# Huvinesh-Rajendran-12/keras-geometric

Hardware: AMD Instinct MI355X
Metric: aggregated edges/sec + achieved HBM GB/s, GCNConv fwd, 1/2/4/8 MI355X (higher is better)
Workload: dtype fp32; 1 GPU; GCNConv fwd, R-MAT 10000000 nodes / 100000000 edges (+self loops), normalized, bias, F 128->128; nodes=10000000, edges=100000000, nodes_per_gpu=10000000, e_agg_per_gpu=110000000, max_in_degree=138539, mode=split-hub, fused aggregate->transform (W on bf16x3-split MFMA, f32-accurate), parallelism=single

## Files before the change

### include/kgx.h

```cpp
#ifndef KGX_H_
#define KGX_H_

#include <stddef.h>
#include <stdint.h>

#ifdef __cplusplus
extern "C" {
#endif

typedef void* kgx_stream_t;

enum kgx_status {
  KGX_OK = 0,
  KGX_ERR_ARG = 1,
  KGX_ERR_HIP = 2,
  KGX_ERR_INDEX = 3,
  KGX_ERR_UNSUPPORTED = 4
};

enum kgx_reduce { KGX_SUM = 0, KGX_MEAN = 1, KGX_MAX = 2, KGX_MIN = 3, KGX_STD = 4 };

enum kgx_epilogue { KGX_EPI_NONE = 0, KGX_EPI_BIAS = 1, KGX_EPI_GIN = 2, KGX_EPI_RAW = 3, KGX_EPI_ACCUM = 4 };

enum kgx_csr_flags {
// ... 92 lines not shown
int kgx_spmm_gemm_ex(int reduce, const int32_t* rowptr, const int32_t* rows, int64_t n_rows,
                     const int32_t* items, int64_t n_items, int64_t n_long_items, const int32_t* split,
                     int64_t n_split, const int32_t* idx, const float* w, const float* x, int64_t ld_x,
                     int64_t F_in, const float* W, int64_t F_out, const float* bias, int flags,
                     float gin_scale, float* out, int64_t ld_out, float* partials, float* agg_out,
                     int64_t ld_agg, kgx_stream_t stream);

int kgx_spmm_gemm_ex2(int reduce, const int32_t* rowptr, const int32_t* rows, int64_t n_rows,
                      const int32_t* items, int64_t n_items, int64_t n_long_items, int64_t n_short_end,
                      const int32_t* tiny_pack, const float* tiny_w, int64_t n_tiny_deg2,
                      const int32_t* split, int64_t n_split,
                      const int32_t* idx, const float* w, const float* x, int64_t ld_x, int64_t F_in,
                      const float* W, int64_t F_out, const float* bias, int flags, float gin_scale, float* out,
                      int64_t ld_out, float* partials, float* agg_out, int64_t ld_agg, kgx_stream_t stream);

int kgx_spmm_gemm_ex3(int reduce, const int32_t* rowptr, const int32_t* rows, int64_t n_rows,
                      const int32_t* items, int64_t n_items, int64_t n_long_items, int64_t n_short_end,
                      const int32_t* tiny_pack, const float* tiny_w, int64_t n_tiny_deg2,
                      const int32_t* split, int64_t n_split, const int32_t* idx, const float* w,
                      const float* x, int64_t ld_x, const float* x2, int64_t n_x1, int64_t F_in,
                      const float* W, int64_t F_out, const float* bias, int flags, float gin_scale, float* out,
                      int64_t ld_out, float* partials, float* agg_out, int64_t ld_agg, kgx_stream_t stream);

int kgx_spmm_gemm_f256(int reduce, const int32_t* rowptr, const int32_t* rows, int64_t n_rows,
                       const int32_t* items, int64_t n_items, int64_t n_long_items, int64_t n_short_end,
                       const int32_t* tiny_pack, const float* tiny_w, const int32_t* split, int64_t n_split,
                       const int32_t* idx, const float* w, const float* x, int64_t ld_x, int64_t F_in,
                       const float* W, int64_t F_out, const float* bias, int flags, float gin_scale,
                       float* out, int64_t ld_out, float* partials, float* agg_out, int64_t ld_agg,
                       kgx_stream_t stream);

int kgx_spmm_gemm_f256_ex(int reduce, const int32_t* rowptr, const int32_t* rows, int64_t n_rows,
                          const int32_t* items, int64_t n_items, int64_t n_long_items, int64_t n_short_end,
                          const int32_t* tiny_pack, const float* tiny_w, const int32_t* split, int64_t n_split,
                          const int32_t* idx, const float* w, const float* x, int64_t ld_x, const float* x2,
                          int64_t n_x1, int64_t F_in, const float* W, int64_t F_out, const float* bias, int flags,
                          float gin_scale, float* out, int64_t ld_out, float* partials, float* agg_out,
                          int64_t ld_agg, kgx_stream_t stream);

int kgx_gemm_tn_workspace_bytes(int64_t N, int64_t K, int64_t M, size_t* bytes);
int kgx_gemm_tn(int64_t N, const float* P, int64_t ldp, int64_t K, const float* D, int64_t ldd, int64_t M,
                float* dW, int64_t ld_dw, float* db, void* workspace, size_t workspace_bytes,
                kgx_stream_t stream);

int kgx_spmm_max_backward(int reduce, int raw, const int32_t* rowptr, int64_t n_rows, const int32_t* idx,
                          const float* table, int64_t ld_table, int64_t F,
// ... 94 lines not shown
```

### keras-geometric_amd/csrc/kgx_internal.h

```cpp
#pragma once

#include <hip/hip_runtime.h>

#include <cstdarg>
#include <cstdint>
#include <cstdio>

#include <cstdlib>
#include <cstring>
#include <mutex>
#include <vector>

#include "kgx.h"

namespace kgx {

void set_error(const char* fmt, ...);

inline hipStream_t as_stream(kgx_stream_t s) { return reinterpret_cast<hipStream_t>(s); }

inline int ceil_log2_u64(uint64_t v) {
  int b = 0;
  while ((uint64_t(1) << b) < v) ++b;
  return b;
// ... 198 lines not shown
  hipStream_t s = nullptr;
  hipError_t fork(CuSplit* c, hipStream_t caller) {
    hipError_t e = hipEventRecord(c->fork, caller);
    if (e == hipSuccess) e = hipStreamWaitEvent(c->head, c->fork, 0);
    if (e == hipSuccess) e = hipStreamWaitEvent(c->tail, c->fork, 0);
    if (e != hipSuccess) return e;
    cs = c;
    s = caller;
    return hipSuccess;
  }
  hipError_t join() {
    if (!cs) return hipSuccess;
    CuSplit* c = cs;
    cs = nullptr;
    const hipError_t e[4] = {hipEventRecord(c->jh, c->head), hipEventRecord(c->jt, c->tail),
                             hipStreamWaitEvent(s, c->jh, 0), hipStreamWaitEvent(s, c->jt, 0)};
    for (hipError_t v : e)
      if (v != hipSuccess) return v;
    return hipSuccess;
  }
  ~SplitJoin() { (void)join(); }
};


inline int next_pow2(int v) {
  int p = 1;
  while (p < v) p <<= 1;
  return p;
}
inline int log2i(int v) {
  int l = 0;
  while ((1 << l) < v) ++l;
  return l;
}

}

#define KGX_CHECK_HIP(expr)                                                      \
  do {                                                                           \
    hipError_t kgx_e_ = (expr);                                                  \
    if (kgx_e_ != hipSuccess) {                                                  \
      kgx::set_error("%s:%d: %s failed: %s", __FILE__, __LINE__, #expr,          \
                     hipGetErrorString(kgx_e_));                                 \
      return KGX_ERR_HIP;                                                        \
    }                                                                            \
  } while (0)
// ... 11 lines not shown
```

### keras-geometric_amd/csrc/spmm_gemm.hip

```cpp
#include <cstdlib>
#include <type_traits>

#include "kgx_bf16x3.h"
#include "kgx_internal.h"
#include "kgx_mfma.h"
#include "kgx_red.h"
#include "kgx_vec.h"

namespace kgx {
namespace {

constexpr int kFin = 128;
constexpr int kGroups = 16;
constexpr int kThreads = kGroups * 32;
constexpr int kTileLd = kFin + 4;

constexpr int kFPlanes = 3;

struct FusedArgs {
  const int32_t* rowptr;
  const int32_t* rows;
  int64_t n_rows;
  const int4* items;
  int64_t n_items;
// ... 6 lines not shown
  int64_t ld_x;
  const float* W;
  int F_in;
  int F_out;
  const float* bias;
  float* out;
  int64_t ld_o;
  float* partials;
  float* agg_out;
  int64_t ld_agg;
  int pre_gin;
  int accumulate;
  int share_gpu;
  int relu;
  float gin_scale;
  int64_t n_short_end;
  const int4* tpack;
  const float2* tw;
  int64_t n_tiny;
  int64_t n_tiny2;
  const float* x2b;
  int32_t n_x1;
  bool cu_split;
};


template <bool NARROW, typename Args>
__device__ __forceinline__ void load_w128(const Args& a, bool w_ok, int n_col, int q, bf16x8_t (&wfh)[4],
                                          bf16x8_t (&wfm)[4], bf16x8_t (&wfl)[4]) {
  auto wv = [&](int k) { return w_ok && (!NARROW || k < a.F_in) ? a.W[int64_t(k) * a.F_out + n_col] : 0.0f; };
#pragma unroll
  for (int s = 0; s < 4; ++s) {
    u32x4_t ph, pm, pl;
#pragma unroll
    for (int j = 0; j < 8; j += 2) {
      const float v0 = wv(32 * q + 8 * s + j), v1 = wv(32 * q + 8 * s + j + 1);
      uint32_t h, m_, l;
      split3_pair(v0, v1, h, m_, l);
      ph[j / 2] = h;
      pm[j / 2] = m_;
      pl[j / 2] = l;
    }
    wfh[s] = __builtin_bit_cast(bf16x8_t, ph);
    wfm[s] = __builtin_bit_cast(bf16x8_t, pm);
    wfl[s] = __builtin_bit_cast(bf16x8_t, pl);
  }
// ... 558 lines not shown
        vload<4>(xv, a.x + int64_t(row) * a.ld_x + (!NARROW || lane * 4 < a.F_in ? lane * 4 : 0));
#pragma unroll
        for (int k = 0; k < 4; ++k) acc[k] = __fadd_rn(__fmul_rn(a.gin_scale, xv[k]), acc[k]);
      }
#pragma unroll
      for (int k = 0; k < 4; ++k) vrow[g][lane * 4 + k] = acc[k];
      if (a.agg_out && (!NARROW || lane * 4 < a.F_in)) vstore<4>(a.agg_out + int64_t(row) * a.ld_agg + lane * 4, acc);
    }
    __syncthreads();
    if (row >= 0) {
      for (int c = lane; c < a.F_out; c += 32) {
        float s = 0.0f;
        for (int k = 0; k < (NARROW ? a.F_in : kFin); ++k) s = fmaf(vrow[g][k], a.W[int64_t(k) * a.F_out + c], s);
        float v = s + (a.bias ? a.bias[c] : 0.0f);
        if (a.accumulate) v = __fadd_rn(a.out[int64_t(row) * a.ld_o + c], v);
        if (a.relu) v = fmaxf(v, 0.0f);
        a.out[int64_t(row) * a.ld_o + c] = v;
      }
    }
    __syncthreads();
  }
}

inline int fused_fork_mode() {
  const char* h = getenv("KGX_FUSED_FORK");
  return h ? atoi(h) : 0;
}

inline unsigned fused_grid(const FusedArgs& a, int64_t need, int64_t full) {
  const int64_t cap = a.share_gpu ? shared_cap(full) : full;
  return unsigned(need < cap ? need : cap);
}

template <int RED, bool W, bool TWO, bool NARROW>
int launch_short(const FusedArgs& a, hipStream_t s, int cus) {
  auto k = spmm_gemm_short_kernel<RED, W, TWO, NARROW>;
  const int64_t need = (a.n_short_end - a.n_long + kShortRows - 1) / kShortRows;
  hipLaunchKernelGGL(k, dim3(fused_grid(a, need, occupancy_blocks(k, kThreads, 2, cus))), dim3(kThreads), 0, s, a);
  KGX_CHECK_LAUNCH();
  return KGX_OK;
}

template <int RED, bool W, bool TWO, bool NARROW>
int launch_tiny(const FusedArgs& a, hipStream_t s, int cus) {
  const bool extra = a.pre_gin || a.agg_out;
  for (int part = 0; part < 2; ++part) {
// ... 1 lines not shown
    b.tpack = a.tpack + (part ? a.n_tiny2 : 0);
    b.tw = a.tw ? a.tw + (part ? a.n_tiny2 : 0) : nullptr;
    b.n_tiny = part ? a.n_tiny - a.n_tiny2 : a.n_tiny2;
    if (b.n_tiny <= 0) continue;
    auto k = part ? (extra ? spmm_gemm_tiny_kernel<RED, W, true, 1, TWO, NARROW>
                           : spmm_gemm_tiny_kernel<RED, W, false, 1, TWO, NARROW>)
                  : (extra ? spmm_gemm_tiny_kernel<RED, W, true, 2, TWO, NARROW>
                           : spmm_gemm_tiny_kernel<RED, W, false, 2, TWO, NARROW>);
    const int rows = part ? tiny_rows<1>() : tiny_rows<2>();
    const int64_t need = (b.n_tiny + rows - 1) / rows;
    hipLaunchKernelGGL(k, dim3(fused_grid(a, need, cus > 0 ? cus : cu_count())), dim3(kTinyThreads), 0, s, b);
    KGX_CHECK_LAUNCH();
  }
  return KGX_OK;
}

template <int RED, bool W, bool TWO = false, bool NARROW = false>
int launch(const FusedArgs& a, hipStream_t s) {
  const int64_t work = a.items ? a.n_long : a.n_rows;
  const bool has_short = a.items && a.n_long < a.n_short_end;
  const bool has_tiny = a.tpack && a.n_tiny > 0;
  hipStream_t sh = s, st = s;
  int cus_h = 0, cus_t = 0;
  SplitJoin join;
  if ((a.cu_split || fused_fork_mode() == 3) && work > 0 && (has_tiny || has_short)) {
    const char* e = getenv("KGX_FUSED_CU_SPLIT");
    if (CuSplit* cs = cu_split(e ? atoi(e) : 8, s)) {
      KGX_CHECK_HIP(join.fork(cs, s));
      sh = cs->head;
      st = cs->tail;
      cus_h = cs->n_head;
      cus_t = cs->n_tail;
    }
  }
  auto k = spmm_gemm_kernel<RED, W, TWO, NARROW>;
  auto fk = spmm_gemm_fixup_kernel<RED, NARROW>;
  if (work > 0) {
    const int64_t need = (work + kGroups - 1) / kGroups;
    hipLaunchKernelGGL(k, dim3(fused_grid(a, need, occupancy_blocks(k, kThreads, 2, cus_h))), dim3(kThreads), 0, sh, a);
    KGX_CHECK_LAUNCH();
  }
  if (has_short && launch_short<RED, W, TWO, NARROW>(a, st, cus_t) != KGX_OK) return KGX_ERR_HIP;
  if (has_tiny && launch_tiny<RED, W, TWO, NARROW>(a, st, cus_t) != KGX_OK) return KGX_ERR_HIP;
  if (a.items && a.n_split > 0) {
    const int64_t blocks = (a.n_split + 7) / 8;
    hipLaunchKernelGGL(fk, dim3(unsigned(blocks < 4096 ? blocks : 4096)), dim3(256), 0, sh, a);
    KGX_CHECK_LAUNCH();
  }
  KGX_CHECK_HIP(join.join());
  return KGX_OK;
}

}
}

using namespace kgx;

extern "C" int kgx_spmm_gemm(int reduce, const int32_t* rowptr, const int32_t* rows, int64_t n_rows,
                             const int32_t* items, int64_t n_items, const int32_t* split, int64_t n_split,
                             const int32_t* idx, const float* w, const float* x, int64_t ld_x, int64_t F_in,
                             const float* W, int64_t F_out, const float* bias, int flags, float gin_scale,
                             float* out, int64_t ld_out, float* partials, float* agg_out, int64_t ld_agg,
                             kgx_stream_t stream_) {
  return kgx_spmm_gemm_ex(reduce, rowptr, rows, n_rows, items, n_items, n_items, split, n_split, idx, w, x, ld_x,
                          F_in, W, F_out, bias, flags, gin_scale, out, ld_out, partials, agg_out, ld_agg, stream_);
}
// ... 10 lines not shown
}

extern "C" int kgx_spmm_gemm_ex2(int reduce, const int32_t* rowptr, const int32_t* rows, int64_t n_rows,
                                 const int32_t* items, int64_t n_items, int64_t n_long_items, int64_t n_short_end,
                                 const int32_t* tiny_pack, const float* tiny_w, int64_t n_tiny_deg2,
                                 const int32_t* split,
                                 int64_t n_split, const int32_t* idx, const float* w, const float* x, int64_t ld_x,
                                 int64_t F_in, const float* W, int64_t F_out, const float* bias, int flags,
                                 float gin_scale, float* out, int64_t ld_out, float* partials, float* agg_out,
                                 int64_t ld_agg, kgx_stream_t stream_) {
  return kgx_spmm_gemm_ex3(reduce, rowptr, rows, n_rows, items, n_items, n_long_items, n_short_end, tiny_pack, tiny_w,
                           n_tiny_deg2, split, n_split, idx, w, x, ld_x, nullptr, 0, F_in, W, F_out, bias, flags,
                           gin_scale, out, ld_out, partials, agg_out, ld_agg, stream_);
}

extern "C" int kgx_spmm_gemm_ex3(int reduce, const int32_t* rowptr, const int32_t* rows, int64_t n_rows,
                                 const int32_t* items, int64_t n_items, int64_t n_long_items, int64_t n_short_end,
                                 const int32_t* tiny_pack, const float* tiny_w, int64_t n_tiny_deg2,
                                 const int32_t* split, int64_t n_split, const int32_t* idx, const float* w,
                                 const float* x, int64_t ld_x, const float* x2, int64_t n_x1, int64_t F_in,
                                 const float* W, int64_t F_out, const float* bias, int flags, float gin_scale,
                                 float* out, int64_t ld_out, float* partials, float* agg_out, int64_t ld_agg,
                                 kgx_stream_t stream_) {
  hipStream_t stream = as_stream(stream_);
  KGX_REQUIRE(!x2 || (n_x1 >= 0 && n_x1 < (int64_t(1) << 31) && reinterpret_cast<uintptr_t>(x2) % 16 == 0),
              KGX_ERR_ARG, "kgx_spmm_gemm: x2 must be 16-byte aligned and 0 <= n_x1 < 2^31");
  KGX_REQUIRE(!x2 || (reduce == KGX_SUM && F_in == kFin && F_out % 16 == 0), KGX_ERR_UNSUPPORTED,
              "kgx_spmm_gemm: two-table gathers are implemented for sums at F_in 128, F_out %% 16 == 0 "
              "(the sharded GCN / GIN passes)");
  KGX_REQUIRE(!items || tiny_pack || n_short_end == n_items, KGX_ERR_ARG,
              "kgx_spmm_gemm: without tiny_pack, n_short_end must equal n_items");
  KGX_REQUIRE(!items || (n_long_items >= 0 && n_long_items <= n_short_end && n_short_end <= n_items), KGX_ERR_ARG,
              "kgx_spmm_gemm: need 0 <= n_long_items <= n_short_end <= n_items");
  KGX_REQUIRE(!tiny_pack || (items && (w == nullptr || tiny_w)), KGX_ERR_ARG,
              "kgx_spmm_gemm: the tiny-row records need the schedule (and weights when weighted)");
  KGX_REQUIRE(!tiny_pack || (n_tiny_deg2 >= 0 && n_tiny_deg2 <= n_items - n_short_end), KGX_ERR_ARG,
              "kgx_spmm_gemm: n_tiny_deg2 must lie in [0, n_items - n_short_end]");
  KGX_REQUIRE(reduce >= KGX_SUM && reduce <= KGX_MIN, KGX_ERR_ARG, "kgx_spmm_gemm: reduce %d unsupported", reduce);
  KGX_REQUIRE(F_in > 0 && F_in <= kFin && F_in % 4 == 0, KGX_ERR_UNSUPPORTED,
              "kgx_spmm_gemm: F_in must be a multiple of 4 <= %d (got %lld)", kFin, (long long)F_in);
  KGX_REQUIRE(F_out > 0 && F_out <= 128 && F_out % 4 == 0, KGX_ERR_UNSUPPORTED,
              "kgx_spmm_gemm: F_out must be a multiple of 4 <= 128 (got %lld)", (long long)F_out);
  KGX_REQUIRE(n_rows >= 0 && n_items >= 0 && n_split >= 0, KGX_ERR_ARG, "kgx_spmm_gemm: negative size");
  KGX_REQUIRE((flags & ~(KGX_FUSED_PRE_GIN | KGX_FUSED_ACCUMULATE | KGX_FUSED_SHARE_GPU | KGX_FUSED_RELU |
                         KGX_FUSED_CU_SPLIT)) == 0,
              KGX_ERR_ARG, "kgx_spmm_gemm: unknown flags 0x%x", flags);
// ... 25 lines not shown
  a.n_split = items ? n_split : 0;
  a.idx = idx;
  a.w = w;
  a.x = x;
  a.ld_x = ld_x;
  a.n_x1 = x2 ? int32_t(n_x1) : INT32_MAX;
  a.x2b = x2 ? reinterpret_cast<const float*>(reinterpret_cast<uintptr_t>(x2) -
                                               uintptr_t(n_x1) * uintptr_t(ld_x) * sizeof(float))
             : x;
  a.W = W;
  a.F_in = int(F_in);
  a.F_out = int(F_out);
  a.bias = bias;
  a.out = out;
  a.ld_o = ld_out;
  a.partials = partials;
  a.agg_out = agg_out;
  a.ld_agg = ld_agg;
  a.pre_gin = (flags & KGX_FUSED_PRE_GIN) != 0;
  a.accumulate = (flags & KGX_FUSED_ACCUMULATE) != 0;
  a.share_gpu = (flags & KGX_FUSED_SHARE_GPU) != 0;
  a.relu = (flags & KGX_FUSED_RELU) != 0;
  a.cu_split = (flags & KGX_FUSED_CU_SPLIT) != 0;
  a.gin_scale = gin_scale;
  const bool wt = w != nullptr;
  if (x2) return wt ? launch<KGX_SUM, true, true>(a, stream) : launch<KGX_SUM, false, true>(a, stream);
  if (F_in < kFin || F_out % 16 != 0) {
    switch (reduce) {
      case KGX_SUM: return wt ? launch<KGX_SUM, true, false, true>(a, stream) : launch<KGX_SUM, false, false, true>(a, stream);
      case KGX_MEAN: return wt ? launch<KGX_MEAN, true, false, true>(a, stream) : launch<KGX_MEAN, false, false, true>(a, stream);
      case KGX_MAX: return wt ? launch<KGX_MAX, true, false, true>(a, stream) : launch<KGX_MAX, false, false, true>(a, stream);
      default: return wt ? launch<KGX_MIN, true, false, true>(a, stream) : launch<KGX_MIN, false, false, true>(a, stream);
    }
  }
  switch (reduce) {
    case KGX_SUM: return wt ? launch<KGX_SUM, true>(a, stream) : launch<KGX_SUM, false>(a, stream);
    case KGX_MEAN: return wt ? launch<KGX_MEAN, true>(a, stream) : launch<KGX_MEAN, false>(a, stream);
    case KGX_MAX: return wt ? launch<KGX_MAX, true>(a, stream) : launch<KGX_MAX, false>(a, stream);
    default: return wt ? launch<KGX_MIN, true>(a, stream) : launch<KGX_MIN, false>(a, stream);
  }
}
```

### keras-geometric_amd/keras_geometric_amd/_native.py

```python

from __future__ import annotations

import ctypes
import os
from pathlib import Path

import torch

_PKG_ROOT = Path(__file__).resolve().parent.parent
LIB_PATH = Path(os.environ.get("KGX_LIB", _PKG_ROOT / "lib" / "libkgx.so"))

KGX_OK, KGX_ERR_ARG, KGX_ERR_HIP, KGX_ERR_INDEX, KGX_ERR_UNSUPPORTED = range(5)
SUM, MEAN, MAX, MIN, STD = range(5)
EPI_NONE, EPI_BIAS, EPI_GIN, EPI_RAW, EPI_ACCUM = range(5)
FUSED_PRE_GIN, FUSED_ACCUMULATE, FUSED_SHARE_GPU, FUSED_RELU, FUSED_CU_SPLIT = 1, 2, 4, 8, 16
CSR_SELF_LOOPS, CSR_SEGMENT_ONLY, CSR_GCN_NORM = 1, 2, 4
DENSE_RELU, DENSE_ACCUMULATE = 1, 2
DENSE_MAX_K, DENSE_MAX_N = 256, 256
POOL_SCORE_TANH = 1
POOL_MAX_F = 256
NEG_NO_SELF, NEG_REJECT_EDGES = 1, 2
EDGE_DOT_U = 8

REDUCE_IDS = {"sum": SUM, "mean": MEAN, "max": MAX, "min": MIN, "std": STD}
# ... 67 lines not shown
        _i32p, _f32p, _f32p, _i64, _i64, _f32p, _i64, _f32p, _int, ctypes.c_float,
        _f32p, _i64, _f32p, _f32p, _i64, ctypes.c_void_p,
    ],
    "kgx_spmm_gemm_ex2": [
        _int, _i32p, _i32p, _i64, _i32p, _i64, _i64, _i64, _i32p, _f32p, _i64, _i32p, _i64,
        _i32p, _f32p, _f32p, _i64, _i64, _f32p, _i64, _f32p, _int, ctypes.c_float,
        _f32p, _i64, _f32p, _f32p, _i64, ctypes.c_void_p,
    ],
    "kgx_spmm_gemm_f256": [
        _int, _i32p, _i32p, _i64, _i32p, _i64, _i64, _i64, _i32p, _f32p, _i32p, _i64,
        _i32p, _f32p, _f32p, _i64, _i64, _f32p, _i64, _f32p, _int, ctypes.c_float,
        _f32p, _i64, _f32p, _f32p, _i64, ctypes.c_void_p,
    ],
    "kgx_spmm_gemm_f256_ex": [
        _int, _i32p, _i32p, _i64, _i32p, _i64, _i64, _i64, _i32p, _f32p, _i32p, _i64,
        _i32p, _f32p, _f32p, _i64, _f32p, _i64, _i64, _f32p, _i64, _f32p, _int, ctypes.c_float,
        _f32p, _i64, _f32p, _f32p, _i64, ctypes.c_void_p,
    ],
    "kgx_spmm_gemm_ex3": [
        _int, _i32p, _i32p, _i64, _i32p, _i64, _i64, _i64, _i32p, _f32p, _i64, _i32p, _i64,
        _i32p, _f32p, _f32p, _i64, _f32p, _i64, _i64, _f32p, _i64, _f32p, _int, ctypes.c_float,
        _f32p, _i64, _f32p, _f32p, _i64, ctypes.c_void_p,
    ],
    "kgx_spmm_max_backward": [
        _int, _int, _i32p, _i64, _i32p, _f32p, _i64, _i64, _f32p, _i64, _f32p, _i64, ctypes.c_void_p,
    ],
    "kgx_gatv2_backward": [
        _i32p, _i32p, _i64, _i32p, _i64, _i32p, _i64, _i32p, _f32p, _f32p, _i64, _f32p, _int, _int,
        ctypes.c_float, _f32p, _i64, _f32p, _f32p, _f32p, _i64,
        _i32p, _i32p, _i64, _i32p, _i64, _i32p, _i64, _i32p, _i32p,
        _f32p, _f32p, _i64, _f32p, _f32p, _f32p, _f32p, _i32p, ctypes.c_float, ctypes.c_uint64, ctypes.c_void_p,
    ],
    "kgx_gatv2": [
        _i32p, _i32p, _i64, _i32p, _i64, _i32p, _i64,
        _i32p, _f32p, _f32p, _i64, _f32p, _int, _int, ctypes.c_float,
        _f32p, _i64, _f32p, _f32p, _f32p, _i32p, ctypes.c_float, ctypes.c_uint64, ctypes.c_void_p,
    ],
    "kgx_softmax_pool": [
        _i32p, _i32p, _i64, _i32p, _i64, _i32p, _i64, _i32p, _f32p, _i64, _i64,
        _f32p, _f32p, _f32p, _int, _f32p, _f32p, _i64, _f32p, _f32p, ctypes.c_void_p,
    ],
    "kgx_softmax_pool_backward": [
        _i64, _i64, _i32p, _f32p, _i64, _i64, _f32p, _f32p, _f32p, _i64, _f32p, _i64, _f32p, _i64, _f32p,
        ctypes.c_void_p,
    ],
    "kgx_dense": [
# ... 103 lines not shown
```

### keras-geometric_amd/keras_geometric_amd/ops.py

```python

from __future__ import annotations

import ctypes
import os
import threading
from typing import List, Optional

import torch

from . import _native as nat
from .graph import CSRGraph


def _f32c(t: Optional[torch.Tensor]) -> Optional[torch.Tensor]:
    if t is None:
        return None
    if t.dtype != torch.float32:
        raise TypeError(f"kgx kernels compute in fp32; got {t.dtype}")
    return t.contiguous()


_EXACT_DYN = __import__("os").environ.get("KGX_EXACT_DYN", "1") != "0"


# ... 229 lines not shown
        return True
    idx = dev.index if dev.index is not None else torch.cuda.current_device()
    ok = _DEVICE_SPLIT_OK.get(idx)
    if ok is None:
        ok = _DEVICE_SPLIT_OK[idx] = nat.lib().kgx_cu_split_supported(int(idx)) == 1
    return ok


def _split_allowed(dev: torch.device | None = None) -> bool:
    if _share_gpu() and os.environ.get("KGX_CU_SPLIT_SHARED") != "1":
        return False
    if getattr(_NOSPLIT, "on", False):
        return False
    if dev is not None and dev.type == "cuda" and dev.index is not None and dev.index != torch.cuda.current_device():
        return False
    return _device_split_ok(dev)


def _count_cu_split() -> None:
    global CU_SPLIT_LAUNCHES
    CU_SPLIT_LAUNCHES += 1


def _fused_cu_split(n_edges: int, n_tail_rows: int) -> bool:
    per32 = _per32_override("KGX_FUSED_CU_SPLIT")
    if per32 is not None:
        return n_tail_rows > 0 and per32 > 0
    return n_edges >= 50_000_000 and n_tail_rows >= 2_000_000


def _partial_width(x: torch.Tensor) -> int:
    return F256 if x.shape[1] == F256 else 128


def _fused_launch(out, agg, x, x2, rowptr, rows, items, split, idx, w, n_slots, reduce, W, bias, flags, gin_scale,
                  allow_split, n_long, tpack, tw, n_short_end, n_tiny2, dev):
    n_dst = rowptr.numel() - 1
    n_items = 0 if items is None else items.shape[0]
    n_split = 0 if split is None else split.shape[0]
    partials = None
    if items is not None and n_split > 0:
        partials = torch.empty((n_slots, _partial_width(x)), dtype=torch.float32, device=dev)
    allow_split = allow_split and items is not None
    if x.shape[1] == F256:
        if tpack is not None and allow_split and _split_allowed(dev) and \
                _f256_cu_split(idx.numel(), n_items - (n_short_end if n_short_end >= 0 else n_items)):
            flags |= nat.FUSED_CU_SPLIT
            _count_cu_split()
        _f256_call(reduce, rowptr, rows, n_dst, items, n_items, split, n_split, idx, w, x, x2, W, bias, flags,
                   gin_scale, out, partials, agg, dev, tpack, tw, n_short_end, n_long)
        return
    n_long = n_items if n_long < 0 or n_long > n_items else n_long
    n_se, tpack, tw, n_tiny2 = _tiny_abi(items, n_items, n_long, tpack, tw if w is not None else None, n_short_end,
                                         n_tiny2)
    if allow_split and _split_allowed(dev) and _fused_cu_split(idx.numel(), n_items - n_long):
        flags |= nat.FUSED_CU_SPLIT
        _count_cu_split()
    x2p, n_x1 = _x2_args(x, x2)
    nat.check(
        nat.lib().kgx_spmm_gemm_ex3(
            reduce, nat.ptr(rowptr), nat.ptr(rows), n_dst, nat.ptr(items), n_items, n_long, n_se, nat.ptr(tpack),
            nat.ptr(tw), n_tiny2, nat.ptr(split), n_split,
            nat.ptr(idx), nat.ptr(w), nat.ptr(x), x.stride(0), x2p, n_x1, x.shape[1], nat.ptr(W), W.shape[1],
            nat.ptr(bias), flags, float(gin_scale), nat.ptr(out), out.stride(0), nat.ptr(partials),
            nat.ptr(agg), agg.stride(0) if agg is not None else 0, nat.stream(dev),
        ),
        "kgx_spmm_gemm",
    )


def _spmm_gemm_impl(x, rowptr, rows, items, split, idx, w, n_slots, reduce, W, bias, pre_gin, gin_scale, save_agg,
                    relu=False, n_long=-1, tpack=None, tw=None, n_short_end=-1, n_tiny2=0, x2=None):
    x, w, W, bias, x2 = _f32c(x), _f32c(w), _f32c(W), _f32c(bias), _f32c(x2)
    dev = nat.require_device(x, rowptr, rows, idx, w, W, bias, items, split, x2)
    n_dst = rowptr.numel() - 1
    out = torch.empty((n_dst, W.shape[1]), dtype=torch.float32, device=dev)
    agg = torch.empty((n_dst if save_agg else 0, x.shape[1]), dtype=torch.float32, device=dev)
    if n_dst == 0:
        return out, agg
    flags = int(pre_gin) | (nat.FUSED_SHARE_GPU if _share_gpu() else 0) | (nat.FUSED_RELU if relu else 0)
    _fused_launch(out, agg if save_agg else None, x, x2, rowptr, rows, items, split, idx, w, n_slots, reduce, W, bias,
                  flags, gin_scale, not save_agg, n_long, tpack, tw, n_short_end, n_tiny2, dev)
    return out, agg


@torch.library.custom_op("kgx::spmm_gemm", mutates_args=())
def spmm_gemm(
    x: torch.Tensor,
    rowptr: torch.Tensor,
    rows: torch.Tensor,
    items: Optional[torch.Tensor],
    split: Optional[torch.Tensor],
    idx: torch.Tensor,
    w: Optional[torch.Tensor],
    n_slots: int,
    reduce: int,
    W: torch.Tensor,
    bias: Optional[torch.Tensor],
    pre_gin: bool,
    gin_scale: float,
    relu: bool = False,
    n_long: int = -1,
    tpack: Optional[torch.Tensor] = None,
    tw: Optional[torch.Tensor] = None,
    n_short_end: int = -1,
# ... 545 lines not shown


def multi_aggregate(g: CSRGraph, table: torch.Tensor, reduces, *, by_edge: bool = False,
                    exact: bool = False) -> torch.Tensor:
    ids = _reduce_list(reduces)
    if _needs_grad(table):
        return _MultiAggregateFn.apply(table, g, ids, bool(by_edge), bool(exact))
    return _multi_aggregate_raw(g, table, ids, by_edge, exact)


def _tiny_of(g, items):
    if items is None:
        return None, None, -1, 0
    from . import tiny

    return tiny.tiny_pack(g)


def _aggregate_transform_raw(g, x, W, red, weighted, bias, pre_gin, gin_scale, exact, relu=False, x2=None):
    items, _, split, _, n_slots = g.work(exact)
    w = g.w if weighted else None
    if weighted and w is None:
        raise ValueError("graph was built without GCN normalisation weights")
    return _timed(lambda: torch.ops.kgx.spmm_gemm(
        x, g.rowptr, g.rows, items, split, g.col, w, n_slots, red, W, bias, bool(pre_gin), float(gin_scale),
        bool(relu), g.n_long if items is not None else -1, *_tiny_of(g, items), x2
    ))


def gemm_tn(P: torch.Tensor, D: torch.Tensor, with_db: bool = False):
    P = P if P.stride(-1) == 1 else P.contiguous()
    D = D if D.stride(-1) == 1 else D.contiguous()
    dev = nat.require_device(P, D)
    if P.dtype != torch.float32 or D.dtype != torch.float32 or P.dim() != 2 or D.dim() != 2 or P.shape[0] != D.shape[0]:
        raise ValueError(f"gemm_tn: float32 [N, K] and [N, M] expected (got {tuple(P.shape)}, {tuple(D.shape)})")
    N, K, M = P.shape[0], P.shape[1], D.shape[1]
    dW = torch.empty((K, M), dtype=torch.float32, device=dev)
    db = torch.empty(M, dtype=torch.float32, device=dev) if with_db else None
    if K == 0 or M == 0:
        return dW, (db.zero_() if db is not None else None)
    L = nat.lib()
    nbytes = ctypes.c_size_t(0)
    nat.check(L.kgx_gemm_tn_workspace_bytes(N, K, M, ctypes.byref(nbytes)), "kgx_gemm_tn_workspace_bytes")
    ws = torch.empty(max(nbytes.value, 4), dtype=torch.uint8, device=dev)
    nat.check(L.kgx_gemm_tn(N, nat.ptr(P), P.stride(0), K, nat.ptr(D), D.stride(0), M, nat.ptr(dW), M, nat.ptr(db),
                            nat.ptr(ws), nbytes.value, nat.stream(dev)), "kgx_gemm_tn")
    return dW, db


class _AggregateTransformFn(torch.autograd.Function):

    @staticmethod
    def forward(ctx, x, W, bias, g, red, weighted, pre_gin, gin_scale, exact):
        ctx.g, ctx.red, ctx.weighted, ctx.pre_gin, ctx.gin_scale, ctx.exact = g, red, weighted, pre_gin, gin_scale, exact
        items, _, split, _, n_slots = g.work(exact)
        w = g.w if weighted else None
        if ctx.needs_input_grad[1]:
            out, P = _timed(lambda: torch.ops.kgx.spmm_gemm_save(
                x, g.rowptr, g.rows, items, split, g.col, w, n_slots, red, W, bias, bool(pre_gin), float(gin_scale),
                g.n_long if items is not None else -1, *_tiny_of(g, items)))
        else:
            out = _aggregate_transform_raw(g, x, W, red, weighted, bias, pre_gin, gin_scale, exact)
            P = None
        ctx.save_for_backward(x if red in (nat.MAX, nat.MIN) else None, W, P)
        ctx.x_rows = x.shape[0]
        return out

    @staticmethod
    def backward(ctx, grad_out):
        from . import graph as G

        x, W, P = ctx.saved_tensors
        grad_out = grad_out.contiguous()
        g_x = g_W = g_b = None
        overlap = ctx.needs_input_grad[1] and ctx.needs_input_grad[0] and grad_out.is_cuda and _tn_overlap()
        W_t = W.t().contiguous() if ctx.needs_input_grad[0] else None
        start = None
        if overlap:
            start = torch.cuda.Event()
            start.record()
        if not overlap and ctx.needs_input_grad[1]:
            g_W, g_b = gemm_tn(P, grad_out, with_db=ctx.needs_input_grad[2])
        elif not ctx.needs_input_grad[1] and ctx.needs_input_grad[2]:
# ... 639 lines not shown
```

### keras-geometric_amd/keras_geometric_amd/tiny.py

```python

from __future__ import annotations

import os
from typing import Optional

import torch

TINY_MAX = 2
_MIN_ROWS = 4096


def tiny_suffix_start(items: torch.Tensor) -> int:
    n = items.shape[0]
    if n == 0:
        return 0
    if items.is_cuda:
        from .graph import schedule_suffixes

        return schedule_suffixes(items, TINY_MAX, TINY_MAX)[1]
    lens = items[:, 2] - items[:, 1]
    big = (lens > TINY_MAX) | (items[:, 3] >= 0)
    nz = torch.nonzero(big)
    return int(nz[-1]) + 1 if nz.numel() else 0

# ... 6 lines not shown
    return pack[:n].long(), (tw[:n] if tw is not None else None)


def _tiny_pack_device(g, its: torch.Tensor, start: int, n: int):
    import ctypes

    from . import _native as nat

    dev = its.device
    pack = torch.empty((n, 4), dtype=torch.int32, device=dev)
    w = getattr(g, "w", None)
    tw = torch.empty((n, 2), dtype=torch.float32, device=dev) if w is not None else None
    ws = torch.empty(16, dtype=torch.uint8, device=dev)
    out = (ctypes.c_int64 * 2)()
    nat.check(nat.lib().kgx_tiny_pack(nat.ptr(its.contiguous()), start, n, nat.ptr(g.col), nat.ptr(w),
                                      int(g.col.numel()), nat.ptr(pack), nat.ptr(tw), nat.ptr(ws), out,
                                      nat.stream(dev)), "kgx_tiny_pack")
    n2, last2 = int(out[0]), int(out[1])
    if n2 and last2 != n2:
        n2 = n
    return pack, tw, start, n2


def tiny_pack(g, refresh: bool = False) -> tuple[Optional[torch.Tensor], Optional[torch.Tensor], int, int]:
    cached = getattr(g, "_kgx_tiny", None)
    w_now = getattr(g, "w", None)
    if cached is not None and not refresh and getattr(g, "_kgx_tiny_w", None) is w_now:
        return cached
    res = (None, None, -1, 0)
    items = getattr(g, "items", None)
    if items is not None and os.environ.get("KGX_TINY", "1") not in ("0", "false", "False"):
        n_items = int(getattr(g, "n_items", items.shape[0]))
        its = items[:n_items]
        start = tiny_suffix_start(its)
        n_long = getattr(g, "n_long", -1)
        start = max(start, n_long if 0 <= n_long <= n_items else 0)
        if n_items - start >= _MIN_ROWS and its.is_cuda and g.col.numel() > 0:
            res = _tiny_pack_device(g, its, start, n_items - start)
        elif n_items - start >= _MIN_ROWS:
            t = its[start:]
            beg = t[:, 1].long()
            deg = (t[:, 2] - t[:, 1]).long()
            last = max(int(g.col.numel()) - 1, 0)
            i0 = beg.clamp(max=last)
            i1 = (beg + (deg > 1).long()).clamp(max=last)
            if g.col.numel() == 0:
                res = (None, None, -1, 0)
                g._kgx_tiny, g._kgx_tiny_w = res, w_now
                return res
            c0 = torch.where(deg > 0, g.col[i0].long(), torch.zeros_like(deg))
            c1 = torch.where(deg > 0, g.col[i1].long(), torch.zeros_like(deg))
            pack = torch.stack([t[:, 0].long(), deg, c0, c1], 1).to(torch.int32).contiguous()
            tw = None
            if getattr(g, "w", None) is not None:
                w0 = torch.where(deg > 0, g.w[i0], torch.zeros_like(g.w[i0]))
                w1 = torch.where(deg > 1, g.w[i1], torch.zeros_like(g.w[i1]))
                tw = torch.stack([w0, w1], 1).to(torch.float32).contiguous()
            n2 = int((deg == 2).sum())
            if n2 and not bool((deg[:n2] == 2).all()):
                n2 = pack.shape[0]
            res = (pack, tw, start, n2)
    try:
        g._kgx_tiny = res
        g._kgx_tiny_w = w_now
    except AttributeError:
        pass
    return res
```

Measured before the change: 12.59 billion edges/s.

## Add cost-model plan to balance fused SpMM-GEMM work across CU-split streams

Adds a byte-based cost model that uses a degree histogram of the work items to choose cut points. Short rows can move to the head stream, or low-degree long rows can move to the tail stream, so the two CU partitions finish at about the same time. The same model decides whether to split at all, in place of fixed edge and row thresholds. This aims to cut idle time when one partition finishes before the other, at the cost of hardcoded per-class rate constants, extra kernel launches, and a one-time host-side histogram pass.

```diff
diff --git a/include/kgx.h b/include/kgx.h
--- a/include/kgx.h
+++ b/include/kgx.h
@@ -138,6 +138,18 @@
                       const float* W, int64_t F_out, const float* bias, int flags, float gin_scale, float* out,
                       int64_t ld_out, float* partials, float* agg_out, int64_t ld_agg, kgx_stream_t stream);
 
+int kgx_spmm_gemm_ex4(int reduce, const int32_t* rowptr, const int32_t* rows, int64_t n_rows,
+                      const int32_t* items, int64_t n_items, int64_t n_long_items, int64_t n_short_end,
+                      const int32_t* tiny_pack, const float* tiny_w, int64_t n_tiny_deg2,
+                      const int32_t* split, int64_t n_split, const int32_t* idx, const float* w,
+                      const float* x, int64_t ld_x, const float* x2, int64_t n_x1, int64_t F_in,
+                      const float* W, int64_t F_out, const float* bias, int flags, float gin_scale, float* out,
+                      int64_t ld_out, float* partials, float* agg_out, int64_t ld_agg,
+                      const int64_t* plan_counts, kgx_stream_t stream);
+
+int kgx_fused_split_plan(const int64_t* counts, int F_in, int F_out, int flags, int store_p, int per32,
+                         int cut_permille, int64_t* out);
+
 int kgx_spmm_gemm_f256(int reduce, const int32_t* rowptr, const int32_t* rows, int64_t n_rows,
                        const int32_t* items, int64_t n_items, int64_t n_long_items, int64_t n_short_end,
                        const int32_t* tiny_pack, const float* tiny_w, const int32_t* split, int64_t n_split,
diff --git a/keras-geometric_amd/csrc/kgx_internal.h b/keras-geometric_amd/csrc/kgx_internal.h
--- a/keras-geometric_amd/csrc/kgx_internal.h
+++ b/keras-geometric_amd/csrc/kgx_internal.h
@@ -244,6 +244,118 @@
   ~SplitJoin() { (void)join(); }
 };
 
+constexpr int kPlanHist = 17;
+constexpr int kPlanCounts = 6 + kPlanHist;
+struct FusedPlanIn {
+  int64_t n_edges;
+  int64_t n_items, n_long, n_short_end;
+  int64_t n_tiny2;
+  int64_t n_chunk;
+  int64_t hist[kPlanHist];
+};
+struct FusedPlan {
+  bool split = false;
+  int64_t cut_s = 0, cut_l = 0;
+  double t_head = 0, t_tail = 0, t_seq = 0, t_split = 0;
+};
+enum { kClsMain = 0, kClsShort = 1, kClsTiny2 = 2, kClsTiny1 = 3 };
+constexpr double kInterference = 1.10;
+constexpr double kSplitMargin = 0.97;
+constexpr double kRateSplit[4][2] = {{31.6, 30.5}, {20.1, 23.2}, {28.5, 30.4}, {24.6, 30.2}};
+constexpr double kRateWhole[4][2] = {{30.2, 30.2}, {20.5, 22.2}, {24.3, 22.6}, {20.4, 20.9}};
+constexpr double kSplitMinSeq = 2.0e-3;
+constexpr int64_t kSplitMinTailRows = 64;
+
+inline double fused_plan_bytes(int64_t rows, int64_t edges, int F_in, int F_out, bool store_p, bool accumulate) {
+  return double(edges) * (4.0 * F_in + 8.0) + double(rows) * 4.0 * F_out * (accumulate ? 2.0 : 1.0) +
+         (store_p ? double(rows) * 4.0 * F_in : 0.0);
+}
+
+inline int64_t fused_plan_low_edges(const FusedPlanIn& c, int64_t rows) {
+  int64_t e = 0;
+  for (int d = 0; d < kPlanHist - 1 && rows > 0; ++d) {
+    const int64_t n = c.hist[d] < rows ? c.hist[d] : rows;
+    e += n * d;
+    rows -= n;
+  }
+  return e;
+}
+
+inline bool fused_plan_counts_ok(const FusedPlanIn& c) {
+  int64_t sum = 0;
+  for (int d = 0; d < kPlanHist; ++d) {
+    if (c.hist[d] < 0) return false;
+    sum += c.hist[d];
+  }
+  return c.n_edges >= 0 && 0 <= c.n_chunk && c.n_chunk <= c.n_long && c.n_long <= c.n_short_end &&
+         c.n_short_end <= c.n_items && c.n_tiny2 >= 0 && c.n_tiny2 <= c.n_items - c.n_short_end &&
+         sum == c.n_items - c.n_chunk && c.n_items - c.n_long <= sum - c.hist[kPlanHist - 1];
+}
+
+constexpr int kPlanCutAuto = 1 << 20;
+inline FusedPlan fused_split_plan(const FusedPlanIn& c, int F_in, int F_out, bool store_p, bool accumulate,
+                                  int cus_head, int cus_tail, int cut_permille = kPlanCutAuto) {
+  FusedPlan p;
+  p.cut_s = c.n_long;
+  p.cut_l = c.n_long;
+  if (!fused_plan_counts_ok(c) || cus_head <= 0 || cus_tail <= 0) return p;
+  const int P = store_p ? 1 : 0;
+  const int64_t n_short = c.n_short_end - c.n_long, n_tiny = c.n_items - c.n_short_end;
+  const int64_t n_tiny1 = n_tiny - c.n_tiny2;
+  int64_t low16 = 0;
+  for (int d = 0; d < kPlanHist - 1; ++d) low16 += c.hist[d];
+  const int64_t movable = low16 - (c.n_items - c.n_long);
+  auto edges_from = [&](int64_t pos) { return fused_plan_low_edges(c, c.n_items - pos); };
+  auto bytes = [&](int64_t a, int64_t b) {
+    return fused_plan_bytes(b - a, edges_from(a) - edges_from(b), F_in, F_out, store_p, accumulate);
+  };
+  const double GB = 1e9;
+  const double b_t1 = bytes(c.n_items - n_tiny1, c.n_items), b_t2 = bytes(c.n_short_end, c.n_items - n_tiny1);
+  const double b_short = bytes(c.n_long, c.n_short_end);
+  const double b_main = fused_plan_bytes(c.n_long, c.n_edges - edges_from(c.n_long), F_in, F_out, store_p, accumulate);
+  const int cus = cus_head + cus_tail;
+  p.t_seq = (b_main / kRateWhole[kClsMain][P] + b_short / kRateWhole[kClsShort][P] +
+             b_t2 / kRateWhole[kClsTiny2][P] + b_t1 / kRateWhole[kClsTiny1][P]) / (GB * cus);
+  auto alone = [&](int cls, double b, int n_cus) { return b / (kRateSplit[cls][P] * kInterference * GB * n_cus); };
+  const double t_tiny = alone(kClsTiny2, b_t2, cus_tail) + alone(kClsTiny1, b_t1, cus_tail);
+  auto legs = [&](int64_t cut_s, int64_t cut_l, double& th, double& tt) {
+    const double bs_head = bytes(c.n_long, cut_s), bl_tail = bytes(cut_l, c.n_long);
+    th = alone(kClsMain, b_main - bl_tail, cus_head) + alone(kClsShort, bs_head, cus_head);
+    tt = alone(kClsShort, b_short - bs_head, cus_tail) + t_tiny + alone(kClsMain, bl_tail, cus_tail);
+  };
+  double th, tt;
+  if (cut_permille >= 0 && cut_permille <= 1000) {
+    p.cut_s = c.n_long + n_short * cut_permille / 1000;
+  } else if (cut_permille < 0 && cut_permille >= -1000) {
+    p.cut_l = c.n_long - movable * (-cut_permille) / 1000;
+  } else {
+    legs(c.n_long, c.n_long, th, tt);
+    if (tt > th) {
+      int64_t lo = 0, hi = n_short;
+      while (lo < hi) {
+        const int64_t mid = lo + (hi - lo) / 2;
+        legs(c.n_long + mid, c.n_long, th, tt);
+        if (th >= tt) hi = mid; else lo = mid + 1;
+      }
+      p.cut_s = c.n_long + lo;
+    } else {
+      int64_t lo = 0, hi = movable;
+      while (lo < hi) {
+        const int64_t mid = lo + (hi - lo) / 2;
+        legs(c.n_long, c.n_long - mid, th, tt);
+        if (tt >= th) hi = mid; else lo = mid + 1;
+      }
+      p.cut_l = c.n_long - lo;
+    }
+  }
+  legs(p.cut_s, p.cut_l, th, tt);
+  p.t_head = th;
+  p.t_tail = tt;
+  p.t_split = kInterference * (th > tt ? th : tt);
+  p.split = c.n_items - c.n_long >= kSplitMinTailRows && c.n_long > 0 && p.t_seq >= kSplitMinSeq &&
+            p.t_split < kSplitMargin * p.t_seq;
+  return p;
+}
 
 inline int next_pow2(int v) {
   int p = 1;
diff --git a/keras-geometric_amd/csrc/spmm_gemm.hip b/keras-geometric_amd/csrc/spmm_gemm.hip
--- a/keras-geometric_amd/csrc/spmm_gemm.hip
+++ b/keras-geometric_amd/csrc/spmm_gemm.hip
@@ -52,6 +52,7 @@
   const float* x2b;
   int32_t n_x1;
   bool cu_split;
+  const int64_t* plan_counts;
 };
 
 
@@ -656,6 +657,27 @@
   }
 }
 
+
+inline int fused_split_cut() {
+  static const int cut = [] {
+    const char* e = getenv("KGX_FUSED_SPLIT_CUT");
+    return e && *e ? atoi(e) : kPlanCutAuto;
+  }();
+  return cut;
+}
+
+inline FusedPlanIn plan_in(const int64_t* c) {
+  FusedPlanIn in;
+  in.n_edges = c[0];
+  in.n_items = c[1];
+  in.n_long = c[2];
+  in.n_short_end = c[3];
+  in.n_tiny2 = c[4];
+  in.n_chunk = c[5];
+  for (int d = 0; d < kPlanHist; ++d) in.hist[d] = c[6 + d];
+  return in;
+}
+
 inline int fused_fork_mode() {
   const char* h = getenv("KGX_FUSED_FORK");
   return h ? atoi(h) : 0;
@@ -703,6 +725,7 @@
   const bool has_tiny = a.tpack && a.n_tiny > 0;
   hipStream_t sh = s, st = s;
   int cus_h = 0, cus_t = 0;
+  int64_t cut_s = a.n_long, cut_l = a.n_long;
   SplitJoin join;
   if ((a.cu_split || fused_fork_mode() == 3) && work > 0 && (has_tiny || has_short)) {
     const char* e = getenv("KGX_FUSED_CU_SPLIT");
@@ -712,17 +735,42 @@
       st = cs->tail;
       cus_h = cs->n_head;
       cus_t = cs->n_tail;
+      if (a.plan_counts) {
+        const FusedPlan p = fused_split_plan(plan_in(a.plan_counts), a.F_in, a.F_out, a.agg_out != nullptr,
+                                             a.accumulate != 0, cus_h, cus_t, fused_split_cut());
+        if (p.cut_s > a.n_long && p.cut_s <= a.n_short_end) cut_s = p.cut_s;
+        if (p.cut_l < a.n_long && p.cut_l >= a.plan_counts[5] && p.cut_l >= 0) cut_l = p.cut_l;
+      }
     }
   }
   auto k = spmm_gemm_kernel<RED, W, TWO, NARROW>;
   auto fk = spmm_gemm_fixup_kernel<RED, NARROW>;
-  if (work > 0) {
-    const int64_t need = (work + kGroups - 1) / kGroups;
-    hipLaunchKernelGGL(k, dim3(fused_grid(a, need, occupancy_blocks(k, kThreads, 2, cus_h))), dim3(kThreads), 0, sh, a);
+  if (work > 0 && (!a.items || cut_l > 0)) {
+    FusedArgs b = a;
+    if (a.items) b.n_long = cut_l;
+    const int64_t need = ((a.items ? cut_l : work) + kGroups - 1) / kGroups;
+    hipLaunchKernelGGL(k, dim3(fused_grid(a, need, occupancy_blocks(k, kThreads, 2, cus_h))), dim3(kThreads), 0, sh, b);
     KGX_CHECK_LAUNCH();
   }
-  if (has_short && launch_short<RED, W, TWO, NARROW>(a, st, cus_t) != KGX_OK) return KGX_ERR_HIP;
+  if (cut_s > a.n_long) {
+    FusedArgs b = a;
+    b.n_short_end = cut_s;
+    if (launch_short<RED, W, TWO, NARROW>(b, sh, cus_h) != KGX_OK) return KGX_ERR_HIP;
+  }
+  if (cut_s < a.n_short_end) {
+    FusedArgs b = a;
+    b.n_long = cut_s;
+    if (launch_short<RED, W, TWO, NARROW>(b, st, cus_t) != KGX_OK) return KGX_ERR_HIP;
+  }
   if (has_tiny && launch_tiny<RED, W, TWO, NARROW>(a, st, cus_t) != KGX_OK) return KGX_ERR_HIP;
+  if (cut_l < a.n_long) {
+    FusedArgs b = a;
+    b.items = a.items + cut_l;
+    b.n_long = a.n_long - cut_l;
+    hipLaunchKernelGGL(k, dim3(fused_grid(b, (b.n_long + kGroups - 1) / kGroups, occupancy_blocks(k, kThreads, 2, cus_t))),
+                       dim3(kThreads), 0, st, b);
+    KGX_CHECK_LAUNCH();
+  }
   if (a.items && a.n_split > 0) {
     const int64_t blocks = (a.n_split + 7) / 8;
     hipLaunchKernelGGL(fk, dim3(unsigned(blocks < 4096 ? blocks : 4096)), dim3(256), 0, sh, a);
@@ -779,6 +827,37 @@
                                  const float* W, int64_t F_out, const float* bias, int flags, float gin_scale,
                                  float* out, int64_t ld_out, float* partials, float* agg_out, int64_t ld_agg,
                                  kgx_stream_t stream_) {
+  return kgx_spmm_gemm_ex4(reduce, rowptr, rows, n_rows, items, n_items, n_long_items, n_short_end, tiny_pack, tiny_w,
+                           n_tiny_deg2, split, n_split, idx, w, x, ld_x, x2, n_x1, F_in, W, F_out, bias, flags,
+                           gin_scale, out, ld_out, partials, agg_out, ld_agg, nullptr, stream_);
+}
+
+extern "C" int kgx_fused_split_plan(const int64_t* counts, int F_in, int F_out, int flags, int store_p, int per32,
+                                    int cut_permille, int64_t* out) {
+  KGX_REQUIRE(counts && out && F_in > 0 && F_out > 0 && per32 > 0 && per32 < 32, KGX_ERR_ARG,
+              "kgx_fused_split_plan: bad arguments");
+  const int cus_tail = 256 * per32 / 32;
+  const FusedPlan p = fused_split_plan(plan_in(counts), F_in, F_out, store_p != 0, (flags & KGX_FUSED_ACCUMULATE) != 0,
+                                       256 - cus_tail, cus_tail, cut_permille);
+  out[0] = p.split ? 1 : 0;
+  out[1] = p.cut_s;
+  out[2] = p.cut_l;
+  out[3] = int64_t(p.t_head * 1e9);
+  out[4] = int64_t(p.t_tail * 1e9);
+  out[5] = int64_t(p.t_seq * 1e9);
+  out[6] = int64_t(p.t_split * 1e9);
+  out[7] = fused_plan_counts_ok(plan_in(counts)) ? 1 : 0;
+  return KGX_OK;
+}
+
+extern "C" int kgx_spmm_gemm_ex4(int reduce, const int32_t* rowptr, const int32_t* rows, int64_t n_rows,
+                                 const int32_t* items, int64_t n_items, int64_t n_long_items, int64_t n_short_end,
+                                 const int32_t* tiny_pack, const float* tiny_w, int64_t n_tiny_deg2,
+                                 const int32_t* split, int64_t n_split, const int32_t* idx, const float* w,
+                                 const float* x, int64_t ld_x, const float* x2, int64_t n_x1, int64_t F_in,
+                                 const float* W, int64_t F_out, const float* bias, int flags, float gin_scale,
+                                 float* out, int64_t ld_out, float* partials, float* agg_out, int64_t ld_agg,
+                                 const int64_t* plan_counts, kgx_stream_t stream_) {
   hipStream_t stream = as_stream(stream_);
   KGX_REQUIRE(!x2 || (n_x1 >= 0 && n_x1 < (int64_t(1) << 31) && reinterpret_cast<uintptr_t>(x2) % 16 == 0),
               KGX_ERR_ARG, "kgx_spmm_gemm: x2 must be 16-byte aligned and 0 <= n_x1 < 2^31");
@@ -850,6 +929,10 @@
   a.share_gpu = (flags & KGX_FUSED_SHARE_GPU) != 0;
   a.relu = (flags & KGX_FUSED_RELU) != 0;
   a.cu_split = (flags & KGX_FUSED_CU_SPLIT) != 0;
+  a.plan_counts = (plan_counts && items && plan_counts[1] == n_items && plan_counts[2] == n_long_items &&
+                   plan_counts[3] == n_short_end && plan_counts[4] == a.n_tiny2)
+                      ? plan_counts
+                      : nullptr;
   a.gin_scale = gin_scale;
   const bool wt = w != nullptr;
   if (x2) return wt ? launch<KGX_SUM, true, true>(a, stream) : launch<KGX_SUM, false, true>(a, stream);
diff --git a/keras-geometric_amd/keras_geometric_amd/_native.py b/keras-geometric_amd/keras_geometric_amd/_native.py
--- a/keras-geometric_amd/keras_geometric_amd/_native.py
+++ b/keras-geometric_amd/keras_geometric_amd/_native.py
@@ -113,6 +113,13 @@
         _i32p, _f32p, _f32p, _i64, _f32p, _i64, _i64, _f32p, _i64, _f32p, _int, ctypes.c_float,
         _f32p, _i64, _f32p, _f32p, _i64, ctypes.c_void_p,
     ],
+    "kgx_spmm_gemm_ex4": [
+        _int, _i32p, _i32p, _i64, _i32p, _i64, _i64, _i64, _i32p, _f32p, _i64, _i32p, _i64,
+        _i32p, _f32p, _f32p, _i64, _f32p, _i64, _i64, _f32p, _i64, _f32p, _int, ctypes.c_float,
+        _f32p, _i64, _f32p, _f32p, _i64, ctypes.POINTER(ctypes.c_int64), ctypes.c_void_p,
+    ],
+    "kgx_fused_split_plan": [ctypes.POINTER(ctypes.c_int64), _int, _int, _int, _int, _int, _int,
+                             ctypes.POINTER(ctypes.c_int64)],
     "kgx_spmm_max_backward": [
         _int, _int, _i32p, _i64, _i32p, _f32p, _i64, _i64, _f32p, _i64, _f32p, _i64, ctypes.c_void_p,
     ],
diff --git a/keras-geometric_amd/keras_geometric_amd/ops.py b/keras-geometric_amd/keras_geometric_amd/ops.py
--- a/keras-geometric_amd/keras_geometric_amd/ops.py
+++ b/keras-geometric_amd/keras_geometric_amd/ops.py
@@ -275,11 +275,54 @@
     CU_SPLIT_LAUNCHES += 1
 
 
-def _fused_cu_split(n_edges: int, n_tail_rows: int) -> bool:
+_PLAN = threading.local()
+
+
+class _plan_counts:
+
+    def __init__(self, g, items):
+        from . import tiny
+
+        self._counts = tiny.plan_counts(g) if items is not None else None
+
+    def __enter__(self):
+        self._old = getattr(_PLAN, "counts", None)
+        _PLAN.counts = self._counts
+
+    def __exit__(self, *exc):
+        _PLAN.counts = self._old
+
+
+def fused_split_plan(counts, f_in: int = 128, f_out: int = 128, flags: int = 0, store_p: bool = False,
+                     per32: int = 8, cut_permille: int = 1 << 20) -> dict:
+    arr = counts if isinstance(counts, ctypes.Array) else (ctypes.c_int64 * len(counts))(*counts)
+    out = (ctypes.c_int64 * 8)()
+    nat.check(nat.lib().kgx_fused_split_plan(arr, int(f_in), int(f_out), int(flags), int(bool(store_p)), int(per32),
+                                             int(cut_permille), out), "kgx_fused_split_plan")
+    return dict(split=bool(out[0]), cut_s=out[1], cut_l=out[2], head_ms=out[3] / 1e6, tail_ms=out[4] / 1e6,
+                seq_ms=out[5] / 1e6, split_ms=out[6] / 1e6, counts_ok=bool(out[7]))
+
+
+def _fused_cu_split(n_edges: int, n_tail_rows: int, counts=None, f_in: int = 128, f_out: int = 128, flags: int = 0,
+                    store_p: bool = False) -> bool:
     per32 = _per32_override("KGX_FUSED_CU_SPLIT")
+    if counts is None and store_p:
+        return False
     if per32 is not None:
         return n_tail_rows > 0 and per32 > 0
-    return n_edges >= 50_000_000 and n_tail_rows >= 2_000_000
+    if counts is None:
+        return n_edges >= 50_000_000 and n_tail_rows >= 2_000_000
+    key = (int(f_in), int(f_out), flags & nat.FUSED_ACCUMULATE, bool(store_p))
+    cache = getattr(counts, "_kgx_split", None)
+    if cache is None:
+        cache = {}
+        try:
+            counts._kgx_split = cache
+        except AttributeError:
+            pass
+    if key not in cache:
+        cache[key] = fused_split_plan(counts, f_in, f_out, flags, store_p)["split"]
+    return cache[key]
 
 
 def _partial_width(x: torch.Tensor) -> int:
@@ -306,17 +349,21 @@
     n_long = n_items if n_long < 0 or n_long > n_items else n_long
     n_se, tpack, tw, n_tiny2 = _tiny_abi(items, n_items, n_long, tpack, tw if w is not None else None, n_short_end,
                                          n_tiny2)
-    if allow_split and _split_allowed(dev) and _fused_cu_split(idx.numel(), n_items - n_long):
+    counts = getattr(_PLAN, "counts", None)
+    if counts is not None and tuple(counts[0:5]) != (idx.numel(), n_items, n_long, n_se, n_tiny2):
+        counts = None
+    if allow_split and _split_allowed(dev) and \
+            _fused_cu_split(idx.numel(), n_items - n_long, counts, x.shape[1], W.shape[1], flags, agg is not None):
         flags |= nat.FUSED_CU_SPLIT
         _count_cu_split()
     x2p, n_x1 = _x2_args(x, x2)
     nat.check(
-        nat.lib().kgx_spmm_gemm_ex3(
+        nat.lib().kgx_spmm_gemm_ex4(
             reduce, nat.ptr(rowptr), nat.ptr(rows), n_dst, nat.ptr(items), n_items, n_long, n_se, nat.ptr(tpack),
             nat.ptr(tw), n_tiny2, nat.ptr(split), n_split,
             nat.ptr(idx), nat.ptr(w), nat.ptr(x), x.stride(0), x2p, n_x1, x.shape[1], nat.ptr(W), W.shape[1],
             nat.ptr(bias), flags, float(gin_scale), nat.ptr(out), out.stride(0), nat.ptr(partials),
-            nat.ptr(agg), agg.stride(0) if agg is not None else 0, nat.stream(dev),
+            nat.ptr(agg), agg.stride(0) if agg is not None else 0, counts, nat.stream(dev),
         ),
         "kgx_spmm_gemm",
     )
@@ -333,7 +380,7 @@
         return out, agg
     flags = int(pre_gin) | (nat.FUSED_SHARE_GPU if _share_gpu() else 0) | (nat.FUSED_RELU if relu else 0)
     _fused_launch(out, agg if save_agg else None, x, x2, rowptr, rows, items, split, idx, w, n_slots, reduce, W, bias,
-                  flags, gin_scale, not save_agg, n_long, tpack, tw, n_short_end, n_tiny2, dev)
+                  flags, gin_scale, True, n_long, tpack, tw, n_short_end, n_tiny2, dev)
     return out, agg
 
 
@@ -925,10 +972,11 @@
     w = g.w if weighted else None
     if weighted and w is None:
         raise ValueError("graph was built without GCN normalisation weights")
-    return _timed(lambda: torch.ops.kgx.spmm_gemm(
-        x, g.rowptr, g.rows, items, split, g.col, w, n_slots, red, W, bias, bool(pre_gin), float(gin_scale),
-        bool(relu), g.n_long if items is not None else -1, *_tiny_of(g, items), x2
-    ))
+    with _plan_counts(g, items):
+        return _timed(lambda: torch.ops.kgx.spmm_gemm(
+            x, g.rowptr, g.rows, items, split, g.col, w, n_slots, red, W, bias, bool(pre_gin), float(gin_scale),
+            bool(relu), g.n_long if items is not None else -1, *_tiny_of(g, items), x2
+        ))
 
 
 def gemm_tn(P: torch.Tensor, D: torch.Tensor, with_db: bool = False):
@@ -959,9 +1007,10 @@
         items, _, split, _, n_slots = g.work(exact)
         w = g.w if weighted else None
         if ctx.needs_input_grad[1]:
-            out, P = _timed(lambda: torch.ops.kgx.spmm_gemm_save(
-                x, g.rowptr, g.rows, items, split, g.col, w, n_slots, red, W, bias, bool(pre_gin), float(gin_scale),
-                g.n_long if items is not None else -1, *_tiny_of(g, items)))
+            with _plan_counts(g, items):
+                out, P = _timed(lambda: torch.ops.kgx.spmm_gemm_save(
+                    x, g.rowptr, g.rows, items, split, g.col, w, n_slots, red, W, bias, bool(pre_gin),
+                    float(gin_scale), g.n_long if items is not None else -1, *_tiny_of(g, items)))
         else:
             out = _aggregate_transform_raw(g, x, W, red, weighted, bias, pre_gin, gin_scale, exact)
             P = None
diff --git a/keras-geometric_amd/keras_geometric_amd/tiny.py b/keras-geometric_amd/keras_geometric_amd/tiny.py
--- a/keras-geometric_amd/keras_geometric_amd/tiny.py
+++ b/keras-geometric_amd/keras_geometric_amd/tiny.py
@@ -52,6 +52,33 @@
     return pack, tw, start, n2
 
 
+PLAN_HIST = 17
+
+
+def _plan_counts(g, its: torch.Tensor, n_long: int, n_short_end: int, n2: int):
+    import ctypes
+
+    n = int(its.shape[0])
+    if n == 0 or not (0 <= n_long <= n_short_end <= n):
+        return None
+    lens = (its[:, 2] - its[:, 1]).long()
+    chunk = its[:, 3] >= 0
+    n_chunk = chunk.sum()
+    pos = torch.arange(n, device=its.device)
+    stray = (chunk & (pos >= n_chunk)).sum()
+    rising = ((lens[1:] > lens[:-1]) & ~chunk[:-1]).sum()
+    hist = torch.bincount(lens.clamp(max=PLAN_HIST - 1)[~chunk], minlength=PLAN_HIST)
+    vals = torch.cat([torch.stack([n_chunk, stray, rising]), hist]).tolist()
+    if vals[1] or vals[2] or vals[0] > n_long:
+        return None
+    return (ctypes.c_int64 * (6 + PLAN_HIST))(int(g.col.numel()), n, n_long, n_short_end, n2, vals[0], *vals[3:])
+
+
+def plan_counts(g):
+    tiny_pack(g)
+    return getattr(g, "_kgx_plan", None)
+
+
 def tiny_pack(g, refresh: bool = False) -> tuple[Optional[torch.Tensor], Optional[torch.Tensor], int, int]:
     cached = getattr(g, "_kgx_tiny", None)
     w_now = getattr(g, "w", None)
@@ -93,6 +120,11 @@
     try:
         g._kgx_tiny = res
         g._kgx_tiny_w = w_now
+        g._kgx_plan = None
+        if items is not None and getattr(g, "col", None) is not None and 0 <= getattr(g, "n_long", -1):
+            n_items = int(getattr(g, "n_items", items.shape[0]))
+            n_se = res[2] if res[0] is not None else n_items
+            g._kgx_plan = _plan_counts(g, items[:n_items], min(g.n_long, n_items), n_se, res[3] if res[0] is not None else 0)
     except AttributeError:
         pass
     return res
```

Measured after the change: 12.74 billion edges/s, median of 6. No clear change (+1.2%).
